# sevagh/xumx-sliCQ

Hardware: AMD Instinct MI355X
Metric: real-time factor (audio-s demixed / wall-s), 44.1 kHz stereo, offline model (higher is better)
Workload: dtype f32; 1 GPU; BASELINE configs[1]: offline model (Bark-262 sliCQT), one 240 s stereo track (10,584,000 samples, 5 chunks) per GPU, Wiener off (mix-phase), seeded synthetic weights; parallelism=one track per rank, 1 rank(s), no data-path collective

## Files before the change

### include/xumx_slicq_hip.h

```cpp
#ifndef XUMX_SLICQ_HIP_H
#define XUMX_SLICQ_HIP_H

#include <stddef.h>
#include <stdint.h>

#ifdef __cplusplus
extern "C" {
#endif

#define XSQ_ABI_VERSION 2

typedef struct xsq_plan xsq_plan;
typedef struct xsq_model xsq_model;

int xsq_abi_version(void);
const char* xsq_last_error(void);
const char* xsq_build_info(void);

int xsq_plan_create(xsq_plan** out, int L, int tr, int nbands, const int32_t* Lg,
                    const int32_t* c, const float* g, const double* gd, const float* tw);
int xsq_plan_destroy(xsq_plan* plan);
int xsq_plan_num_blocks(const xsq_plan* plan);
int xsq_plan_set_fft_backend(xsq_plan* plan, int backend);
int xsq_plan_set_band_radix4(xsq_plan* plan, int on);
int xsq_plan_set_short_inline(xsq_plan* plan, int on);
int xsq_plan_set_packed_fft(xsq_plan* plan, int on);
int xsq_plan_block_table(const xsq_plan* plan, int64_t* table);
int64_t xsq_plan_coefs_per_slice(const xsq_plan* plan);
int xsq_plan_num_slices(const xsq_plan* plan, int64_t n);

size_t xsq_slicqt_forward_workspace(xsq_plan* plan, int BC, int64_t n);
int xsq_slicqt_forward(xsq_plan* plan, const float* x, int BC, int64_t n, float* coef,
                       void* workspace, size_t workspace_bytes, void* stream);
int xsq_slicqt_forward_xin(xsq_plan* plan, const float* x, int BC, int64_t n, float* coef, float* xin,
                           const float* mean, const float* scale, int split,
                           void* workspace, size_t workspace_bytes, void* stream);

int xsq_slicqt_forward_rows(xsq_plan* plan, const float* x, const int64_t* x_row_offsets, int BC, int64_t n,
                            int64_t n_pad, float* coef, float* xin, const float* mean, const float* scale, int split,
                            void* workspace, size_t workspace_bytes, void* stream);
// ... 204 lines not shown
```

### xumx_slicq_amd/_lib.py

```python
from __future__ import annotations

import ctypes as C
import os

import torch

_HERE = os.path.dirname(os.path.abspath(__file__))
LIB_PATH = os.environ.get("XSQ_LIB") or os.path.join(_HERE, "libxumx_slicq_hip.so")


class XsqError(RuntimeError):
    pass


def _load():
    if not os.path.exists(LIB_PATH):
        raise XsqError(
            f"{LIB_PATH} is missing: the HIP extension is the product path and has no CPU "
            "fallback. Build it with `python -c 'import __graft_entry__ as g; g.build()'` "
            "or `make -C xumx_slicq_amd/csrc`.")
    return C.CDLL(LIB_PATH, mode=C.RTLD_GLOBAL)


lib = _load()

_vp = C.c_void_p
_i32p = C.POINTER(C.c_int32)
_i64p = C.POINTER(C.c_int64)

_SIGS = {
    "xsq_abi_version": (C.c_int, []),
    "xsq_last_error": (C.c_char_p, []),
    "xsq_build_info": (C.c_char_p, []),
    "xsq_plan_create": (C.c_int, [C.POINTER(_vp), C.c_int, C.c_int, C.c_int, _vp, _vp, _vp, _vp, _vp]),
    "xsq_plan_destroy": (C.c_int, [_vp]),
    "xsq_plan_num_blocks": (C.c_int, [_vp]),
    "xsq_plan_set_fft_backend": (C.c_int, [_vp, C.c_int]),
    "xsq_plan_set_band_radix4": (C.c_int, [_vp, C.c_int]),
    "xsq_plan_set_short_inline": (C.c_int, [_vp, C.c_int]),
    "xsq_plan_set_packed_fft": (C.c_int, [_vp, C.c_int]),
    "xsq_plan_block_table": (C.c_int, [_vp, _vp]),
    "xsq_plan_coefs_per_slice": (C.c_int64, [_vp]),
    "xsq_plan_num_slices": (C.c_int, [_vp, C.c_int64]),
    "xsq_slicqt_forward_workspace": (C.c_size_t, [_vp, C.c_int, C.c_int64]),
    "xsq_slicqt_forward": (C.c_int, [_vp, _vp, C.c_int, C.c_int64, _vp, _vp, C.c_size_t, _vp]),
    "xsq_slicqt_forward_xin": (C.c_int, [_vp, _vp, C.c_int, C.c_int64, _vp, _vp, _vp, _vp, C.c_int, _vp, C.c_size_t, _vp]),
    "xsq_slicqt_forward_rows": (C.c_int, [_vp, _vp, _vp, C.c_int, C.c_int64, C.c_int64, _vp, _vp, _vp, _vp, C.c_int, _vp, C.c_size_t, _vp]),
    "xsq_slicqt_forward_rows_indirect": (C.c_int, [_vp, _vp, _vp, _vp, C.c_int, C.c_int64, C.c_int64, _vp, _vp, _vp, _vp, C.c_int, _vp, C.c_size_t, _vp]),
    "xsq_slicqt_inverse_workspace": (C.c_size_t, [_vp, C.c_int, C.c_int]),
    "xsq_slicqt_inverse": (C.c_int, [_vp, _vp, C.c_int, C.c_int, C.c_int64, _vp, _vp, C.c_size_t, _vp]),
    "xsq_slicqt_inverse_rows": (C.c_int, [_vp, _vp, C.c_int, C.c_int, C.c_int64, _vp, _vp, _vp, C.c_size_t, _vp]),
    "xsq_slicqt_inverse_masked": (C.c_int, [_vp, _vp, _vp, C.c_int, C.c_int, C.c_int, C.c_int64, _vp, _vp, _vp, C.c_size_t, _vp]),
    "xsq_slicqt_remix_workspace": (C.c_size_t, [_vp, C.c_int, C.c_int, C.c_int, C.c_int]),
    "xsq_slicqt_inverse_remix": (C.c_int, [_vp, _vp, _vp, _vp, _vp, C.c_int, C.c_int, C.c_int, C.c_int64, _vp, _vp, _vp, C.c_size_t, _vp]),
# ... 148 lines not shown
```

### xumx_slicq_amd/csrc/cdae.hip

```cpp
#include <algorithm>
#include <cmath>
#include <cstdlib>
#include <cstring>
#include <vector>

#include "../../include/xumx_slicq_hip.h"
#include "gemm_tile.h"
#include "gemm_tile_bf3.h"
#include "gemm_tile_bf6.h"
#include "plan.h"
#include "prof.h"

#include "cdae_api.h"

namespace xsq {

__global__ __launch_bounds__(256) void k_magnitude_whiten(const float4* __restrict__ X, float4* __restrict__ xin,
                                                           const int64_t* __restrict__ cum,
                                                           const CdaeBlockDev* __restrict__ blocks,
                                                           const float* __restrict__ mean,
                                                           const float* __restrict__ scale, int nblocks,
                                                           int BC, int S, int64_t nquads, int split) {
    __shared__ int64_t cum_s[128];
    for (int i = threadIdx.x; i < nblocks && i < 128; i += 256) cum_s[i] = cum[i];
// ... 860 lines not shown
extern "C" int xsq_debug_w4_stamps(unsigned long long* out, int reset) {
    XSQ_HIP(hipDeviceSynchronize());
    XSQ_HIP(hipMemcpyFromSymbol(out, HIP_SYMBOL(xsq::g_w4_stamps), 8 * sizeof(unsigned long long)));
    if (reset) { unsigned long long z[8] = {0}; XSQ_HIP(hipMemcpyToSymbol(HIP_SYMBOL(xsq::g_w4_stamps), z, sizeof(z))); }
    return XSQ_OK;
}
#endif

int xsq_model_set_wiener_options(xsq_model* Mo, int softmask, int residual) {
    XSQ_REQUIRE(Mo, "xsq_model_set_wiener_options: null model");
    Mo->wiener_flags = (softmask ? XSQ_WIENER_SOFTMASK : 0) | (residual ? XSQ_WIENER_RESIDUAL : 0);
    return XSQ_OK;
}

int xsq_model_set_winograd(xsq_model* Mo, int on) {
    XSQ_REQUIRE(Mo && on >= 0 && on <= 15, "xsq_model_set_winograd: null model or mask %d (1 = layers 2 / 3 Winograd F(2, 4), 2 / 4 = layer 1 / 4 F(2, 2), 8 = F(4, 4) for long rows)", on);
    XSQ_REQUIRE(!(on & 8) || Mo->wino4, "xsq_model_set_winograd: bit 8 (F(4, 4)) needs a model created with XSQ_WINO4=1 in the environment");
    Mo->winograd = on;
    return XSQ_OK;
}

int xsq_model_destroy(xsq_model* Mo) {
    if (!Mo) return XSQ_OK;
    for (auto& kv : Mo->tiles) (void)hipFree(kv.second.d_tiles);
    (void)hipFree(Mo->d_pool); (void)hipFree(Mo->d_upool); (void)hipFree(Mo->d_pool_split); (void)hipFree(Mo->d_mean); (void)hipFree(Mo->d_scale);
    (void)hipFree(Mo->d_blocks); (void)hipFree(Mo->d_cum); (void)hipFree(Mo->d_blockF);
    delete Mo;
    return XSQ_OK;
}

size_t xsq_cdae_workspace(const xsq_model* Mo, int Bn, int S) {
// ... 15 lines not shown
                       (const float4*)X, (float4*)xin, Mo->d_cum, Mo->d_blocks, mean, scale, Mo->nblocks, Bn * 2, S,
                       total / 4, split);
    return XSQ_OK;
}

template <class T>
static void launch_tiles(void (*kernel)(CdaeArgs, const T*, int), int threads, const CdaeArgs& a, const TileTable& tt, hipStream_t stream) {
    if (tt.ntiles) hipLaunchKernelGGL(kernel, dim3(tt.ntiles), dim3(threads), 0, stream, a, (const T*)tt.d_tiles, tt.ntiles);
}

template <bool TRANSPOSED>
static auto slab_kernel(bool bf3, bool bf6) {
    return bf3 ? cdae_slab_kernel<TRANSPOSED, 1> : bf6 ? cdae_slab_kernel<TRANSPOSED, 2> : cdae_slab_kernel<TRANSPOSED, 3, true>;
}

int cdae_launch_layer(xsq_model* Mo, int layer, const CdaeArgs& a, hipStream_t stream, const char* prof_name) {
    if (layer == 1 || layer == 4)
        for (const CdaeBlockDev& d : Mo->blocks)
            XSQ_REQUIRE(std::max((int64_t)4 * 2 * a.Bn * d.F * a.S * d.T, layer == 4 ? (int64_t)4 * CS * a.Bn * a.T1 * d.F1 : 0) < ((int64_t)1 << 30),
                        "xsq_cdae_forward: B=%d S=%d: a block's layer-%d input exceeds 2^30 bytes; split the batch", a.Bn, a.S, layer);
    if (layer == 4 && !a.gx8)
        for (const CdaeBlockDev& d : Mo->blocks)
            XSQ_REQUIRE((int64_t)2 * a.Bn * d.F * a.S * d.T < ((int64_t)1 << 31),
                        "xsq_cdae_forward: B=%d S=%d overflows the 32-bit offsets of a block; split the batch", a.Bn, a.S);
    if (layer == 4 && a.gx8) layer = 6;

    const bool bf3 = a.split != 0;
    const bool bf1 = Mo->precision == 3;
    const bool bf6 = Mo->precision == 2 || bf1;
    const bool inference = !a.raw && !a.xin8 && !a.gx8;
    const bool fp32 = inference && !bf3 && !bf6;
// ... 133 lines not shown
```

### xumx_slicq_amd/csrc/cdae_api.h

```cpp
#pragma once
#include <map>
#include <mutex>
#include <tuple>
#include <vector>

#include "common.h"
#include "plan.h"

namespace xsq {

static const int H1 = 50, H2 = 51, CS = 52;
static const int NT = 4;

struct CdaeBlockDev {
    int F, T, hop, kf, F1, F2;
    int cumF1, cumF2;
    int ld1, ld4;
    int64_t cum;
    int64_t cumF;
    int64_t w1[NT], w2[NT], w3[NT], w4[NT];
    int64_t s1[NT], s2[NT], s3[NT], b4[NT];
    int64_t u2[NT], u3[NT];
    int64_t u1[NT];
    int nch1, pad_;
// ... 34 lines not shown
    const float* pool;
    const float* xin;
    float* act1;
    float* act2;
    float* act3;
    const float* X;
    float* Y;
    float* masks;
    int Bn, S, T1, T2, causal;
    int raw;
    const float* xin8;
    float* gx8;
    int split = 0;
    const float* poolB = nullptr;
    const float* upool = nullptr;
};


int cdae_launch_layer(xsq_model* Mo, int layer, const CdaeArgs& a, hipStream_t stream, const char* prof_name = nullptr);
int cdae_launch_magnitude(const xsq_model* Mo, const float* X, float* xin, const float* mean, const float* scale,
                          int Bn, int S, hipStream_t stream, int split = 0);

int wiener_em_backward(int nblocks, const int32_t* F, const int32_t* T, const float* X, const float* Y0, const float* masks,
                       float* G, int Bn, int S, int win_len, int batch_group, const void* stats, void* bstats, hipStream_t stream,
                       float* gM = nullptr);
int loss_forward_backward(int nblocks, const int32_t* F, const int32_t* T, const float* pred, const float* target,
                          const float* masks, int Bn, int S, double* out, float* gY, float* gM, void* ws, hipStream_t stream);
int sdr_loss(const float* pred, const float* target, int R, int64_t n, float scale, double* out, float* gy, void* ws, hipStream_t stream);

}
// ... 1 lines not shown
```

### xumx_slicq_amd/csrc/cdae_l4f.h

```cpp
#pragma once
#include "cdae_api.h"
#include "gemm_tile.h"

#ifndef XSQ_L4F_WAVES_PER_EU
#define XSQ_L4F_WAVES_PER_EU 3
#endif
#ifndef XSQ_L4F_SCHED
#define XSQ_L4F_SCHED 0
#endif
#ifndef XSQ_L4F_ABL
#define XSQ_L4F_ABL 0
#endif

namespace xsq {

constexpr int L4_PAIRS = 64;
constexpr int L4_BLD = 56;
constexpr int L4_BROWS = 3 * 64;

__host__ __device__ constexpr int l4f_cols(int W) { return (W + 15) / 16 * 16; }
__host__ __device__ constexpr int l4f_tap_floats(int W) { return 3 * CS * l4f_cols(W); }
__host__ __device__ constexpr int l4f_u_off(int W, int n0, int j, int n, int ci) {
    return 3 * CS * n0 + (j * (l4f_cols(W) - n0 < 64 ? l4f_cols(W) - n0 : 64) + (n - n0)) * CS + ci;
}
// ... 202 lines not shown
        load_a(o, addr_of(pr, 0));
        store_b();
        __syncthreads();
        for (int it = 0; it < run; ++it) {
            const bool more = it + 1 < run;
            const Pair nxp = pair_of(more ? it + 1 : it);
            const Addr nx = addr_of(nxp, 0);
            clear_acc();
            contract(o, nx, more);
            epilogue(pr);
            pr = nxp;
        }
        return;
    }
    if constexpr (NCB <= 2) {
        Ops o;
        const Pair pr = pair_of(0);
        clear_acc();
        load_b(0);
        load_a(o, addr_of(pr, 0));
        for (int df = 0; df < kf; ++df) {
            if (df > 0) __syncthreads();
            store_b();
            __syncthreads();
            const bool more = df + 1 < kf;
            if (more) load_b(df + 1);
            contract(o, addr_of(pr, more ? df + 1 : df), more);
        }
        epilogue(pr);
    }
}

template <bool WITH_Y>
__global__ __launch_bounds__(256, XSQ_L4F_WAVES_PER_EU) void cdae_l4f_kernel(CdaeArgs a, const L4fTileDev* __restrict__ tiles, int ntiles) {
#ifndef XSQ_L4F_LDS_ROWS
#define XSQ_L4F_LDS_ROWS L4_BROWS
#endif
    __shared__ __attribute__((aligned(16))) float Bs[XSQ_L4F_LDS_ROWS * L4_BLD];
    const L4fTileDev t = tiles[xcd_remap(blockIdx.x, ntiles)];
    asm volatile("" :: "s"(t.Q0), "s"(t.kf), "s"(t.F), "s"(t.run), "s"(t.in_off), "s"(t.out_off), "s"(t.bias_off), "s"(t.u_off),
// ... 10 lines not shown
```

### xumx_slicq_amd/csrc/cdae_slab.h

```cpp
#pragma once
#include "cdae_api.h"
#include "gemm_tile_bf3.h"
#include "gemm_tile_bf6.h"

#ifndef XSQ_SLAB_PROLOGUE_PRIO
#define XSQ_SLAB_PROLOGUE_PRIO 0
#endif
#ifndef XSQ_SLAB_STAMP
#define XSQ_SLAB_STAMP 0
#endif
#ifndef XSQ_SLAB_PRIO
#define XSQ_SLAB_PRIO 0
#endif
#ifndef XSQ_SLAB_ABL
#define XSQ_SLAB_ABL 0
#endif

namespace xsq {

constexpr int SLAB_ROWS = 256;
constexpr int SLAB_MAXSEG = 4;
constexpr int SLAB_POS = SLAB_ROWS + 3 * SLAB_MAXSEG;
constexpr int SLAB_KRUN = 4 * CS;
constexpr int SLAB_BLD = 36;
// ... 190 lines not shown
    }
    const int b16_frag = (32 + (lane & 15)) * BLD + 4 * q16;
    const int bv_frag = 48 * BLD + 8 * lk;
    f32x4_t acc16[2] = {{0.f, 0.f, 0.f, 0.f}, {0.f, 0.f, 0.f, 0.f}};
    constexpr int NV = TRANSPOSED ? H1 - 48 : H2 - 48;
    float accv[4] = {0.f, 0.f, 0.f, 0.f};

    constexpr int NKS = 7;
#if XSQ_SLAB_PRIO == 1
    if (__builtin_amdgcn_readfirstlane(tid) >= 256) __builtin_amdgcn_s_setprio(1);
#endif
#if XSQ_SLAB_STAMP
    if (a_base == -12345 || a16_base[0] == -12345 || a16_base[1] == -12345 || s_p0 == -12345) __builtin_trap();
    if (TRANSPOSED && tid == 0 && blockIdx.x < SLAB_STAMP_TILES) g_slab_stamps[blockIdx.x * 8 + 7] = __builtin_amdgcn_s_memrealtime();
#endif
    load_slab(0);
    load_b(0, 0, 0);
    XSQ_SS2(1);
#if XSQ_SLAB_STAMP
    if (sa[0].x == 1.2345e-30f) __builtin_trap();
    XSQ_SS2(2);
#endif
    store_slab();
    store_b(0, 0);
#if XSQ_SLAB_STAMP
    stamp_loads = false;
#endif
    load_b(1, 0, 1);
    load_b(0, 0, 2);
    if (kf > 1 && !LATE) load_slab(1);
#if XSQ_SLAB_PROLOGUE_PRIO
    __builtin_amdgcn_s_setprio(0);
#endif
    __syncthreads();
    XSQ_SS(1);
#if XSQ_SLAB_STAMP
    unsigned long long fetch_t = 0;
#endif
    for (int df = 0; df < kf; ++df) {
        const bool more = df + 1 < kf;
#pragma unroll
        for (int ks = 0; ks < 8; ++ks) {
            if (ks < NKS) {
                if constexpr (LATE && EARLY2) { if (ks == NKS - 1 && more) load_slab(df + 1, 0, XSQ_SLAB_EARLY2 == 1 ? 2 : XSQ_SLAB_EARLY2); }
                const unsigned* Bb = Bs + (ks & 1) * SLAB_BN * BLD;
#pragma unroll
                for (int c = 0; c < 2; ++c) {
                    const int k = 32 * ks + 16 * c;
                    if (k < SLAB_KRUN) {
                        if constexpr (MODE == 3) {
#if XSQ_SLAB_PRIO == 2
                            __builtin_amdgcn_s_setprio(1);
#endif
                            const float* Bf = reinterpret_cast<const float*>(Bb);
                            const float4 alo = *reinterpret_cast<const float4*>(&slabF[a_base + k]);
// ... 74 lines not shown
            } else if (more) {
                if constexpr (LATE) {
#if XSQ_SLAB_STAMP
                    const unsigned long long f0 = __builtin_amdgcn_s_memrealtime();
#endif
                    if constexpr (EARLY2) { load_slab(df + 1, XSQ_SLAB_EARLY2 == 1 ? 2 : XSQ_SLAB_EARLY2, NLD); store_slab(0, NLD); }
                    else {
                        load_slab(df + 1, 0, 4); store_slab(0, 4);
                        load_slab(df + 1, 4, NLD); store_slab(4, NLD);
                    }
#if XSQ_SLAB_STAMP
                    fetch_t += __builtin_amdgcn_s_memrealtime() - f0;
#endif
                } else {
                    store_slab();
                    if (df + 2 < kf) load_slab(df + 2);
                }
            }
            if (ks + 1 < NKS) store_b((ks + 1) & 1, (ks + 1) & 1);
            else if (ks + 1 == 8 && more) store_b(0, 0);
            if (ks + 3 < NKS) load_b((ks + 3) & 1, df, ks + 3);
            else if (ks + 3 >= 8 && more) load_b((ks + 3) & 1, df + 1, ks + 3 - 8);
            __syncthreads();
        }
    }
#undef XSQ_MF
    XSQ_SS(2);
#if XSQ_SLAB_STAMP
    if (TRANSPOSED && tid == 0 && blockIdx.x < SLAB_STAMP_TILES) {
        g_slab_stamps[blockIdx.x * 8 + 4] = kf; g_slab_stamps[blockIdx.x * 8 + 5] = fetch_t;
        g_slab_stamps[blockIdx.x * 8 + 6] = (unsigned)__builtin_amdgcn_s_getreg((4) | (0 << 6) | (31 << 11));
// ... 25 lines not shown
```

### xumx_slicq_amd/csrc/cdae_wino.h

```cpp
#pragma once
#include "cdae_api.h"
#include "gemm_tile.h"

#ifndef XSQ_WINO_WAVES_PER_EU
#define XSQ_WINO_WAVES_PER_EU 2
#endif
#ifndef XSQ_WINO_RAW_AHEAD
#define XSQ_WINO_RAW_AHEAD 0
#endif
#ifndef XSQ_WINO_SWAP
#define XSQ_WINO_SWAP 1
#endif
#ifndef XSQ_WINO_SCHED
#define XSQ_WINO_SCHED 0
#endif
#ifndef XSQ_WINO_SCHED2
#define XSQ_WINO_SCHED2 -1
#endif
#ifndef XSQ_WINO_ABL
#define XSQ_WINO_ABL 0
#endif

namespace xsq {

// ... 155 lines not shown
        f.w[2] = *reinterpret_cast<const float4*>(&Bt[bf + 32 * WN_BLD]);
#pragma unroll
        for (int cc = 0; cc < NV; ++cc) f.u[cc] = Bt[bv + cc * WN_BLD];
        if (tail) {
            const int tb = q * WN_BLD + 16 + kq;
            f.wt[0] = Bt[tb]; f.wt[1] = Bt[tb + 16 * WN_BLD]; f.wt[2] = Bt[tb + 32 * WN_BLD];
#pragma unroll
            for (int cc = 0; cc < NV; ++cc) f.ut[cc] = Bt[(48 + cc) * WN_BLD + 16 + kq];
        }
    };

    const int f0 = t.Q0 / P, q0 = t.Q0 - f0 * P;
    const int npairs = min(WN_PAIRS, Fo * P - t.Q0);
    const int n0 = min(npairs, P - q0);
    int cnt = 0;
    load_chunk(0, 0);
    setup_staging(f0, q0, npairs, n0);
    load_slab(0);
    store_slab();
    store_chunk(0, 0);
    __syncthreads();
    WN_STAMP(0);

    {
        const int myseg = pl >= n0 ? 1 : 0;
        const int eb = (pl + 2 * myseg) * WN_SLD + 4 * kq;
        const int ob = PLANE_O + (pl + myseg) * WN_SLD + 4 * kq;
        float4 dn[5];
        auto read_raw = [&](int s) {
            dn[0] = *reinterpret_cast<const float4*>(&slab[eb + 16 * s]);
            dn[1] = *reinterpret_cast<const float4*>(&slab[ob + 16 * s]);
            dn[2] = *reinterpret_cast<const float4*>(&slab[eb + WN_SLD + 16 * s]);
            dn[3] = *reinterpret_cast<const float4*>(&slab[ob + WN_SLD + 16 * s]);
            dn[4] = *reinterpret_cast<const float4*>(&slab[eb + 2 * WN_SLD + 16 * s]);
        };
        clear_acc();
        for (int df = 0; df < kf; ++df) {
            const bool more = df + 1 < kf;
            if (XSQ_WINO_RAW_AHEAD) read_raw(0);
#pragma unroll
            for (int s = 0; s < 3; ++s) {
                const int cur = cnt & 1;
                if (s < 2) load_chunk(df, s + 1);
                else if (more) { load_chunk(df + 1, 0); load_slab(df + 1); }
                const float* Bc = Bs + cur * 5 * WN_BTILE;
                if (!XSQ_WINO_RAW_AHEAD) read_raw(s);
                Frag fr[2];
                read_frag(fr[0], Bc, s == 2);
                float v[5][4], vt[5];
                {
                    const float d[5][4] = {{dn[0].x, dn[0].y, dn[0].z, dn[0].w}, {dn[1].x, dn[1].y, dn[1].z, dn[1].w}, {dn[2].x, dn[2].y, dn[2].z, dn[2].w},
                                           {dn[3].x, dn[3].y, dn[3].z, dn[3].w}, {dn[4].x, dn[4].y, dn[4].z, dn[4].w}};
#pragma unroll
// ... 171 lines not shown
```

### xumx_slicq_amd/csrc/plan.h

```cpp
#pragma once
#include <algorithm>
#include <map>
#include <mutex>
#include <tuple>
#include <vector>

#include <rocfft/rocfft.h>

#include "common.h"

namespace xsq {

struct FftPlan {
    rocfft_plan plan = nullptr;
    rocfft_execution_info info = nullptr;
    size_t work_bytes = 0;
};

struct TileTable {
    TileDev* d_tiles = nullptr;
    int ntiles = 0;
};

enum class TileKind { BandGemm, Dft4Full, CdaeGemm, CdaeSlab, CdaeWino, CdaeL1f, CdaeL4f };
struct TileKey {
    TileKind kind;
    int rows, S;
    int sub, flags;
    bool operator<(const TileKey& o) const {
        return std::tie(kind, rows, S, sub, flags) < std::tie(o.kind, o.rows, o.S, o.sub, o.flags);
    }
};

template <class D, class T>
static int upload(D*& dst, const T* src, size_t count) {
    dst = nullptr;
    if (!count) return XSQ_OK;
    XSQ_HIP(hipMalloc((void**)&dst, count * sizeof(T)));
    const hipError_t e = hipMemcpy(dst, src, count * sizeof(T), hipMemcpyHostToDevice);
// ... 42 lines not shown
    int band_radix4 = 1;
    void* d_bands4 = nullptr;
    float* d_pool4f = nullptr;
    float* d_pool4i = nullptr;
    int nbands4 = 0;
    std::vector<unsigned char> bands4_host;
    int64_t d4_max_block = 0;
    std::vector<int> bands4_m, bands4_small;
    int fft_backend = 0;
    float2* d_T = nullptr;
    unsigned short* d_tgt16 = nullptr;
    int* d_tgt = nullptr;
    int phase_begin[5] = {0, 0, 0, 0, 0};
    int packed_fft = 0;
    int short_inline = 0;
    void *d_s_item1 = nullptr, *d_s_tw1 = nullptr;
    int *d_s_item2 = nullptr, *d_s_tgt = nullptr;
    float* d_s_wd = nullptr;
    int short_n1 = 0, short_n2 = 0, short_nent = 0, short_sc0 = 0;
    int short_begin[5] = {0, 0, 0, 0, 0};
    int phase_long[4] = {0, 0, 0, 0};
    float* d_tw = nullptr;
    float* d_Wf = nullptr;
    float* d_Wi = nullptr;
    xsq::BandDev* d_bands = nullptr;
    int* d_cov_ptr = nullptr;
    int* d_cov_band = nullptr;
    std::vector<int32_t> h_Lg, h_c;
    std::vector<double> h_gd;
    size_t wf_floats = 0, pool4_floats = 0;
// ... 9 lines not shown
```

### xumx_slicq_amd/csrc/slicqt.hip

```cpp
#include <algorithm>
#include <cmath>
#include <cstdarg>
#include <cstdio>
#include <cstdlib>
#include <cstring>

#include "../../include/xumx_slicq_hip.h"
#include "gemm_tile.h"
#include "plan.h"
#include "prof.h"
#include "slice_fft.h"
#include "band_dft4.h"
#include "band_dft4s.h"

namespace xsq {

static thread_local char g_err[1024] = "";
void set_error(const char* fmt, ...) {
    va_list ap;
    va_start(ap, fmt);
    vsnprintf(g_err, sizeof(g_err), fmt, ap);
    va_end(ap);
}

// ... 259 lines not shown
    float* d = a.dst + base * ((int64_t)a.R * a.nch) + (int64_t)ch * per + e;
#pragma unroll
    for (int r = 0; r < 4; ++r) {
        if (r >= a.R) break;
        float4 acc = make_float4(0.f, 0.f, 0.f, 0.f);
#pragma unroll
        for (int t = 0; t < 4; ++t) {
            if (!a.use[t]) continue;
            const float g = a.g[r][t];
            acc.x = acc.x + g * m[t].x; acc.y = acc.y + g * m[t].y; acc.z = acc.z + g * m[t].z; acc.w = acc.w + g * m[t].w;
        }
        *reinterpret_cast<float4*>(d + (int64_t)r * a.nch * per) = acc;
    }
}

static int get_band_tiles(xsq_plan* P, int rows, TileTable* out) {
    const bool r4 = P->band_radix4 && P->nbands4 > 0;
    return cached_tiles<TileDev>(P->mu, P->tiles, TileKey{TileKind::BandGemm, rows, 0, 0, r4 ? 1 : 0}, out, [&](std::vector<TileDev>& t) {
        if (r4) {
            for (int i = (int)P->bands4_small.size() - 1; i >= 0; --i)
                push_group_tiles(t, P->bands4_small[i], rows, 2 * P->bands[P->bands4_small[i]].Lg);
        } else {
            for (int j = P->nbands - 1; j >= 0; --j) push_group_tiles(t, j, rows, 2 * P->bands[j].Lg);
        }
    });
}

#ifndef XSQ_D4_MIN_LG_DEFAULT
#define XSQ_D4_MIN_LG_DEFAULT 24
#endif

struct Switches {
    bool d4_sym = true;
    int d4_min_lg = XSQ_D4_MIN_LG_DEFAULT;
    Switches() {
        if (const char* e = getenv("XSQ_D4_SYM")) d4_sym = atoi(e) != 0;
        if (const char* e = getenv("XSQ_D4_MIN_LG")) d4_min_lg = atoi(e) >= 16 ? atoi(e) : d4_min_lg;
    }
};
static const Switches& switches() { static const Switches sw; return sw; }
// ... 500 lines not shown
    XSQ_HIP(hipMemcpyFromSymbol(host, HIP_SYMBOL(g_fft_stamps), (size_t)(rows < FFT_STAMP_ROWS ? rows : FFT_STAMP_ROWS) * 64));
    return XSQ_OK;
}
#endif

int xsq_plan_set_packed_fft(xsq_plan* P, int on) {
    XSQ_REQUIRE(P, "xsq_plan_set_packed_fft: null plan");
#if !XSQ_PACKED_FFT_KERNELS
    XSQ_REQUIRE(!on, "xsq_plan_set_packed_fft: this library is built without the packed-fp32 slice FFT kernels "
                "(diagnostic build: make PACKED_FFT=1)");
#endif
    P->packed_fft = on ? 1 : 0;
    return XSQ_OK;
}

int xsq_plan_set_short_inline(xsq_plan* P, int on) {
    XSQ_REQUIRE(P, "xsq_plan_set_short_inline: null plan");
    P->short_inline = on ? 1 : 0;
    return XSQ_OK;
}

int xsq_plan_set_fft_backend(xsq_plan* P, int backend) {
    XSQ_REQUIRE(P && (backend == 0 || backend == 1), "xsq_plan_set_fft_backend: backend must be 0 (auto) or 1 (rocFFT)");
    P->fft_backend = backend;
    return XSQ_OK;
}

int xsq_plan_block_table(const xsq_plan* P, int64_t* table) {
    XSQ_REQUIRE(P && table, "xsq_plan_block_table: null argument");
    for (int b = 0; b < P->nblocks; ++b) {
// ... 100 lines not shown
        XSQ_PROF(adj ? "adjoint_slice_rfft" : "slice_rfft", stream);
        auto kernel = k_slice_rfft<512>;
#if XSQ_PACKED_FFT_KERNELS
        if (P->packed_fft) kernel = k_slice_rfft<512, true>;
#endif
        if (ring) kernel = k_slice_rfft<512, false, true>;
        hipLaunchKernelGGL(kernel, dim3(rows), dim3(512), 0, stream, x, d_tw, fft_tables(P), (float2*)U, S, n, P->h, x_rows, x_slot, s0, ring,
                           const_cast<float*>(x), fresh.x, fresh.first, fresh.stride);
    } else {
        { XSQ_PROF(adj ? "adjoint_slice_window" : "slice_window", stream);
        hipLaunchKernelGGL(k_slice_window, dim3((P->L + 255) / 256, rows), dim3(256), 0, stream, x, d_tw, seg,
                           S, n, P->L, P->h, x_rows, x_slot, s0, ring, const_cast<float*>(x), fresh.x, fresh.first, fresh.stride); }
        { XSQ_PROF(adj ? "adjoint_rfft_L" : "rfft_L", stream); rc = run_fft(f, seg, U, fwork, stream); }
        if (rc) return rc;
    }
    TileTable tt;
    rc = get_band_tiles(P, rows, &tt);
    if (rc) return rc;
    BandFwdOp op{U, coef, P->d_bands, d_Wf, BC, S, P->nbins, P->L, xin, mean, scale, split};
    if (P->band_radix4 && P->nbands4) {
        Band4Args a4{(const Band4Dev*)P->d_bands4, d_pool4f, U, coef, BC, S, P->nbins, P->L, 0, nullptr, 0, xin, mean, scale, split};
        XSQ_PROF(adj ? "adjoint_band_dft4" : "band_analysis_dft4", stream);
        if ((rc = launch_dft4<true>(P, a4, rows, 0, stream))) return rc;
    }
    if (tt.ntiles) { XSQ_PROF(adj ? "adjoint_band_gemm" : "band_analysis_gemm", stream);
    hipLaunchKernelGGL((grouped_gemm_kernel<BandFwdOp>), dim3(tt.ntiles), dim3(256), 0, stream, op,
                       tt.d_tiles, tt.ntiles); }
    XSQ_HIP(hipGetLastError());
    return XSQ_OK;
}

int xsq_slicqt_adjoint_window(int L, int nbands, const int32_t* Lg, const int32_t* c, const double* gd, double* out) {
    XSQ_REQUIRE(Lg && c && gd && out, "xsq_slicqt_adjoint_window: null argument");
    XSQ_REQUIRE(L > 0 && L % 4 == 0 && nbands >= 1, "xsq_slicqt_adjoint_window: L=%d nbands=%d", L, nbands);
    int64_t off = 0;
    for (int j = 0; j < nbands; ++j) {
        const int n = Lg[j];
        XSQ_REQUIRE(n > 0 && n % 2 == 0, "xsq_slicqt_adjoint_window: band %d has Lg=%d", j, n);
        for (int q = 0; q < n; ++q) {
            const int k = c[j] + (q < n / 2 ? q : q - n);
            const double w = (k < 0 || k > L / 2) ? 0.0 : ((k == 0 || k == L / 2) ? 1.0 : 2.0);
            out[off + q] = w * (double)n * (double)n * gd[off + q] / (double)L;
// ... 120 lines not shown
    hipStream_t stream = (hipStream_t)stream_;
    const int rows = BC * S;
    FftPlan f;
    int rc = lds_fft(P) ? XSQ_OK : get_fft(P, 1, rows, &f);
    if (rc) return rc;
    char* w = (char*)ws;
    float* Z = (float*)w;    w += al256((size_t)rows * P->sumFT * 8);
    float2* fr = (float2*)w; if (!lds_fft(P)) w += al256((size_t)rows * P->nbins * 8);
    float* seg = (float*)w;  if (!lds_fft(P)) w += al256((size_t)rows * P->L * 4);
    void* fwork = w;
    if ((size_t)(w - (char*)ws) + f.work_bytes > ws_bytes) {
        set_error("xsq_slicqt_inverse: workspace too small (%zu needed, %zu given)",
                  (size_t)(w - (char*)ws) + f.work_bytes, ws_bytes);
        return XSQ_ERR_WORKSPACE;
    }
    TileTable tt;
    rc = get_band_tiles(P, rows, &tt);
    if (rc) return rc;
    BandInvOp op{coef, Z, P->d_bands, P->d_Wi, BC, S, lds_fft(P) ? (int)P->sumFT : 0, mask, BCx};
    if (P->band_radix4 && P->nbands4) {
        Band4Args a4{(const Band4Dev*)P->d_bands4, P->d_pool4i, coef, Z, BC, S, P->nbins, P->L,
                     lds_fft(P) ? (int)P->sumFT : 0, mask, BCx, nullptr, nullptr, nullptr, 0};
        XSQ_PROF("band_synthesis_dft4", stream);
        if ((rc = launch_dft4<false>(P, a4, rows, mask ? BCx * S : 0, stream))) return rc;
    }
    const bool inl = lds_fft(P) && P->band_radix4 && P->short_inline && P->short_n1 > 0 && !carry;
    if (tt.ntiles && !inl) { XSQ_PROF("band_synthesis_gemm", stream);
    hipLaunchKernelGGL((grouped_gemm_kernel<BandInvOp>), dim3(tt.ntiles), dim3(256), 0, stream, op,
                       tt.d_tiles, tt.ntiles); }
    if (lds_fft(P)) {
        XSQ_PROF("slice_irfft_ola", stream);
        GatherSched G;
        G.tgt = P->d_tgt; G.tgt16 = P->d_tgt16; G.row_len = (int)P->sumFT;
        for (int i = 0; i < 5; ++i) G.begin[i] = P->phase_begin[i];
        for (int i = 0; i < 4; ++i) G.lo[i] = inl ? P->phase_long[i] : P->phase_begin[i];
        ShortSched SS;
        memset(&SS, 0, sizeof(SS));
        if (inl) {
            SS.item1 = (const ShortItem1*)P->d_s_item1; SS.tw1 = (const float2*)P->d_s_tw1; SS.item2 = P->d_s_item2;
            SS.stgt = P->d_s_tgt; SS.swd = P->d_s_wd;
            SS.n1 = P->short_n1; SS.n2 = P->short_n2; SS.nent = P->short_nent; SS.sc0 = P->short_sc0;
            for (int i = 0; i < 5; ++i) SS.begin[i] = P->short_begin[i];
        }
        const ShortIn SI{coef, mask, BC, mask ? BCx : BC};
// ... 126 lines not shown
```

### xumx_slicq_amd/transforms.py

```python
from __future__ import annotations

import ctypes as C
from typing import List

import numpy as np
import torch
import torch.nn as nn
from torch import Tensor

from . import _lib
from .arena import BlockTable
from .plan import SliCQPlan, build_plan


def make_filterbanks(nsgt_base, sample_rate=44100.0):
    if sample_rate != 44100.0:
        raise ValueError("i was lazy and harcoded a lot of 44100.0, forgive me")
    return NSGT_SL(nsgt_base), INSGT_SL(nsgt_base)


class SliCQEngine:

    def __init__(self, plan: SliCQPlan):
        self.plan = plan
# ... 20 lines not shown
        for h in self._handles.values():
            _lib.check(_lib.lib.xsq_plan_set_band_radix4(h, int(self._band_radix4)), "xsq_plan_set_band_radix4")

    def set_packed_fft(self, on: bool):
        on = bool(on)
        if on == getattr(self, "_packed_fft", False):
            return
        for h in self._handles.values():
            _lib.check(_lib.lib.xsq_plan_set_packed_fft(h, int(on)), "xsq_plan_set_packed_fft")
        self._packed_fft = on

    def set_short_inline(self, on: bool):
        self._short_inline = bool(on)
        for h in self._handles.values():
            _lib.check(_lib.lib.xsq_plan_set_short_inline(h, int(self._short_inline)), "xsq_plan_set_short_inline")

    def handle(self, device: torch.device):
        if device.type != "cuda":
            raise _lib.XsqError(
                f"the sliCQT runs on a ROCm device only (got a tensor on '{device}'); there is no CPU fallback")
        idx = device.index if device.index is not None else torch.cuda.current_device()
        h = self._handles.get(idx)
        if h is None:
            p = self.plan
            out = C.c_void_p()
            with torch.cuda.device(idx):
                _lib.check(_lib.lib.xsq_plan_create(
                    C.byref(out), p.L, p.tr, p.nbands,
                    p.Lg.ctypes.data, p.c.ctypes.data, p.g.ctypes.data, p.gd.ctypes.data, p.tw.ctypes.data),
                    "xsq_plan_create")
            h = out
            _lib.check(_lib.lib.xsq_plan_set_fft_backend(h, self._fft_backend), "xsq_plan_set_fft_backend")
            _lib.check(_lib.lib.xsq_plan_set_band_radix4(h, int(getattr(self, "_band_radix4", True))),
                       "xsq_plan_set_band_radix4")
            _lib.check(_lib.lib.xsq_plan_set_short_inline(h, int(getattr(self, "_short_inline", False))),
                       "xsq_plan_set_short_inline")
            _lib.check(_lib.lib.xsq_plan_set_packed_fft(h, int(getattr(self, "_packed_fft", False))), "xsq_plan_set_packed_fft")
            self._handles[idx] = h
        return h

    def demixer(self, device: torch.device):
        idx = device.index if device.index is not None else torch.cuda.current_device()
        d = self.__dict__.setdefault("_demixers", {}).get(idx)
        if d is None:
            h = self.handle(device)
            out = C.c_void_p()
            with torch.cuda.device(idx):
                _lib.check(_lib.lib.xsq_demixer_create(C.byref(out), h), "xsq_demixer_create")
            d = self._demixers[idx] = out
        return d

    def workspace(self, device: torch.device, nbytes: int) -> Tensor:
# ... 168 lines not shown
```

Baseline: 55530 x real-time.

## Add register-resident MFMA kernel for short bands and skip dead CDAE border taps

Result: no change. 55890 x real-time (median of 6 runs) (+0.7%).

```diff
diff --git a/include/xumx_slicq_hip.h b/include/xumx_slicq_hip.h
--- a/include/xumx_slicq_hip.h
+++ b/include/xumx_slicq_hip.h
@@ -24,6 +24,7 @@
 int xsq_plan_set_fft_backend(xsq_plan* plan, int backend);
 int xsq_plan_set_band_radix4(xsq_plan* plan, int on);
 int xsq_plan_set_short_inline(xsq_plan* plan, int on);
+int xsq_plan_set_short_mfma(xsq_plan* plan, int on);
 int xsq_plan_set_packed_fft(xsq_plan* plan, int on);
 int xsq_plan_block_table(const xsq_plan* plan, int64_t* table);
 int64_t xsq_plan_coefs_per_slice(const xsq_plan* plan);
diff --git a/xumx_slicq_amd/_lib.py b/xumx_slicq_amd/_lib.py
--- a/xumx_slicq_amd/_lib.py
+++ b/xumx_slicq_amd/_lib.py
@@ -38,6 +38,7 @@
     "xsq_plan_set_fft_backend": (C.c_int, [_vp, C.c_int]),
     "xsq_plan_set_band_radix4": (C.c_int, [_vp, C.c_int]),
     "xsq_plan_set_short_inline": (C.c_int, [_vp, C.c_int]),
+    "xsq_plan_set_short_mfma": (C.c_int, [_vp, C.c_int]),
     "xsq_plan_set_packed_fft": (C.c_int, [_vp, C.c_int]),
     "xsq_plan_block_table": (C.c_int, [_vp, _vp]),
     "xsq_plan_coefs_per_slice": (C.c_int64, [_vp]),
diff --git a/xumx_slicq_amd/csrc/band_short.h b/xumx_slicq_amd/csrc/band_short.h
--- /dev/null
+++ b/xumx_slicq_amd/csrc/band_short.h
@@ -0,0 +1,136 @@
+#pragma once
+#include <type_traits>
+
+#include "common.h"
+#include "gemm_tile.h"
+
+namespace xsq {
+
+constexpr int BS_MAX_LG = 24;
+constexpr int BS_RT = 2;
+constexpr int BS_RUN = 2;
+constexpr int BS_STEP = 64 * BS_RT;
+constexpr int BS_ROWS = BS_STEP * BS_RUN;
+
+template <int NC, class Op>
+__device__ __forceinline__ void band_short_body(const Op& op, const BandDev& b, const int j, const int m0) {
+#pragma clang fp contract(off)
+    constexpr bool FWD = std::is_same<Op, BandFwdOp>::value;
+    const int lane = threadIdx.x & 63, wave = threadIdx.x >> 6;
+    const int q = lane & 15, kq = lane >> 4;
+    const int N = 2 * b.Lg, M = op.BC * op.S, S = op.S;
+    if (m0 + 16 * BS_RT * wave >= M) return;
+
+    float4 w[NC][NC];
+    {
+        const float* W = op.W + b.w_off;
+#pragma unroll
+        for (int nb = 0; nb < NC; ++nb)
+#pragma unroll
+            for (int c = 0; c < NC; ++c)
+                w[nb][c] = 16 * nb + q < N ? *reinterpret_cast<const float4*>(W + (int64_t)(16 * nb + q) * b.ldw + 16 * c + 4 * kq)
+                                           : make_float4(0.f, 0.f, 0.f, 0.f);
+    }
+    float mu = 0.f, sc = 1.f;
+    if constexpr (FWD) { if (op.xin) { mu = op.mean[j]; sc = op.scale[j]; } }
+    const int64_t base = 2 * ((int64_t)op.BC * S * b.cum + (int64_t)b.f * S * b.Lg);
+
+    struct Row { const float* p; const float* mk; int64_t out; bool ok; };
+    auto row_of = [&](int m) {
+        Row r;
+        r.ok = m < M;
+        const int bc = m / S, s = m - bc * S;
+        const int64_t off = base + ((int64_t)bc * b.F * S + s) * N;
+        r.mk = nullptr;
+        if constexpr (FWD) {
+            r.p = op.U + (int64_t)m * 2 * op.nbins;
+            r.out = off;
+        } else {
+            r.out = op.row_len ? 2 * ((int64_t)m * op.row_len + b.ent) : off;
+            if (!op.mask) r.p = op.coef + off;
+            else {
+                r.mk = op.mask + off / 2;
+                r.p = op.coef + 2 * ((int64_t)op.BCx * S * b.cum + (int64_t)b.f * S * b.Lg) + ((int64_t)(bc % op.BCx) * b.F * S + s) * N;
+            }
+        }
+        return r;
+    };
+
+#pragma unroll 1
+    for (int it = 0; it < BS_RUN; ++it) {
+        const int mw = m0 + BS_STEP * it + 16 * BS_RT * wave;
+        if (mw >= M) break;
+        Row r[BS_RT];
+        float4 v[BS_RT][NC];
+        float2 mk[BS_RT][NC];
+#pragma unroll
+        for (int t = 0; t < BS_RT; ++t) {
+            r[t] = row_of(mw + 16 * t + q);
+#pragma unroll
+            for (int c = 0; c < NC; ++c) {
+                const int k = 16 * c + 4 * kq;
+                const bool ok = r[t].ok && k < N;
+                if constexpr (FWD) {
+                    int i0 = b.bin0 + (k >> 1), i1 = i0 + 1;
+                    i0 = i0 < 0 ? -i0 : (i0 > op.L / 2 ? op.L - i0 : i0);
+                    i1 = i1 < 0 ? -i1 : (i1 > op.L / 2 ? op.L - i1 : i1);
+                    const float2 x0 = *reinterpret_cast<const float2*>(ok ? r[t].p + 2 * i0 : zero16());
+                    const float2 x1 = *reinterpret_cast<const float2*>(ok ? r[t].p + 2 * i1 : zero16());
+                    v[t][c] = make_float4(x0.x, x0.y, x1.x, x1.y);
+                } else {
+                    v[t][c] = *reinterpret_cast<const float4*>(ok ? r[t].p + k : zero16());
+                    if (op.mask) mk[t][c] = *reinterpret_cast<const float2*>(ok ? r[t].mk + (k >> 1) : zero16());
+                }
+            }
+        }
+#pragma unroll
+        for (int t = 0; t < BS_RT; ++t) {
+            f32x4 acc[NC];
+#pragma unroll
+            for (int nb = 0; nb < NC; ++nb) acc[nb] = f32x4{0.f, 0.f, 0.f, 0.f};
+#pragma unroll
+            for (int c = 0; c < NC; ++c) {
+                float4 xv = v[t][c];
+                if constexpr (!FWD) {
+                    if (op.mask) { xv.x *= mk[t][c].x; xv.y *= mk[t][c].x; xv.z *= mk[t][c].y; xv.w *= mk[t][c].y; }
+                }
+                const float x[4] = {xv.x, xv.y, xv.z, xv.w};
+#pragma unroll
+                for (int i = 0; i < 4; ++i)
+#pragma unroll
+                    for (int nb = 0; nb < NC; ++nb) {
+                        const float wv[4] = {w[nb][c].x, w[nb][c].y, w[nb][c].z, w[nb][c].w};
+                        acc[nb] = __builtin_amdgcn_mfma_f32_16x16x4f32(wv[i], x[i], acc[nb], 0, 0, 0);
+                    }
+            }
+#pragma unroll
+            for (int nb = 0; nb < NC; ++nb) {
+                const int n = 16 * nb + 4 * kq;
+                if (!r[t].ok || n >= N) continue;
+                const float4 y = make_float4(acc[nb][0], acc[nb][1], acc[nb][2], acc[nb][3]);
+                if constexpr (FWD) {
+                    *reinterpret_cast<float4*>(op.coef + r[t].out + n) = y;
+                    if (op.xin) {
+                        float v0 = whiten_mag(y.x, y.y, mu, sc), v1 = whiten_mag(y.z, y.w, mu, sc);
+                        if (op.split) { v0 = bf3_word(v0); v1 = bf3_word(v1); }
+                        *reinterpret_cast<float2*>(op.xin + ((r[t].out + n) >> 1)) = make_float2(v0, v1);
+                    }
+                } else {
+                    *reinterpret_cast<float4*>(op.Z + r[t].out + n) = y;
+                }
+            }
+        }
+    }
+}
+
+template <class Op>
+__global__ __launch_bounds__(256) void band_short_kernel(const Op op, const TileDev* __restrict__ tiles, int ntiles) {
+    const TileDev t = tiles[blockIdx.x];
+    const BandDev b = op.bands[t.group];
+    const int nc = (2 * b.Lg + 15) >> 4;
+    if (nc == 2) band_short_body<2>(op, b, t.group, t.m0);
+    else if (nc == 3) band_short_body<3>(op, b, t.group, t.m0);
+    else band_short_body<1>(op, b, t.group, t.m0);
+}
+
+}
diff --git a/xumx_slicq_amd/csrc/cdae.hip b/xumx_slicq_amd/csrc/cdae.hip
--- a/xumx_slicq_amd/csrc/cdae.hip
+++ b/xumx_slicq_amd/csrc/cdae.hip
@@ -898,7 +898,8 @@
 }
 
 int xsq_model_set_winograd(xsq_model* Mo, int on) {
-    XSQ_REQUIRE(Mo && on >= 0 && on <= 15, "xsq_model_set_winograd: null model or mask %d (1 = layers 2 / 3 Winograd F(2, 4), 2 / 4 = layer 1 / 4 F(2, 2), 8 = F(4, 4) for long rows)", on);
+    XSQ_REQUIRE(Mo && on >= 0 && on <= 31, "xsq_model_set_winograd: null model or mask %d (1 = layers 2 / 3 Winograd F(2, 4), 2 / 4 = layer 1 / 4 F(2, 2), 8 = F(4, 4) for long rows, "
+                "16 = layers 3 / 4 visit their dead border taps)", on);
     XSQ_REQUIRE(!(on & 8) || Mo->wino4, "xsq_model_set_winograd: bit 8 (F(4, 4)) needs a model created with XSQ_WINO4=1 in the environment");
     Mo->winograd = on;
     return XSQ_OK;
@@ -944,7 +945,9 @@
     return bf3 ? cdae_slab_kernel<TRANSPOSED, 1> : bf6 ? cdae_slab_kernel<TRANSPOSED, 2> : cdae_slab_kernel<TRANSPOSED, 3, true>;
 }
 
-int cdae_launch_layer(xsq_model* Mo, int layer, const CdaeArgs& a, hipStream_t stream, const char* prof_name) {
+int cdae_launch_layer(xsq_model* Mo, int layer, const CdaeArgs& args, hipStream_t stream, const char* prof_name) {
+    CdaeArgs a = args;
+    a.all_taps = (Mo->winograd & 16) ? 1 : 0;
     if (layer == 1 || layer == 4)
         for (const CdaeBlockDev& d : Mo->blocks)
             XSQ_REQUIRE(std::max((int64_t)4 * 2 * a.Bn * d.F * a.S * d.T, layer == 4 ? (int64_t)4 * CS * a.Bn * a.T1 * d.F1 : 0) < ((int64_t)1 << 30),
diff --git a/xumx_slicq_amd/csrc/cdae_api.h b/xumx_slicq_amd/csrc/cdae_api.h
--- a/xumx_slicq_amd/csrc/cdae_api.h
+++ b/xumx_slicq_amd/csrc/cdae_api.h
@@ -72,6 +72,7 @@
     int split = 0;
     const float* poolB = nullptr;
     const float* upool = nullptr;
+    int all_taps = 0;
 };
 
 
diff --git a/xumx_slicq_amd/csrc/cdae_l4f.h b/xumx_slicq_amd/csrc/cdae_l4f.h
--- a/xumx_slicq_amd/csrc/cdae_l4f.h
+++ b/xumx_slicq_amd/csrc/cdae_l4f.h
@@ -240,16 +240,23 @@
         return;
     }
     if constexpr (NCB <= 2) {
+        int df_lo = 0, df_hi = kf - 1;
+        if (!a.all_taps) {
+            const int R0 = t.Q0 / P, R1 = (min(t.Q0 + L4_PAIRS, a.Bn * F * P) - 1) / P;
+            const int b0 = R0 / F, b1 = R1 / F;
+            const int lo = max(0, R0 - b0 * F - F1 + 1), hi = min(kf - 1, R1 - b1 * F);
+            if (b0 == b1 && lo <= hi) { df_lo = lo; df_hi = hi; }
+        }
         Ops o;
         const Pair pr = pair_of(0);
         clear_acc();
-        load_b(0);
-        load_a(o, addr_of(pr, 0));
-        for (int df = 0; df < kf; ++df) {
-            if (df > 0) __syncthreads();
+        load_b(df_lo);
+        load_a(o, addr_of(pr, df_lo));
+        for (int df = df_lo; df <= df_hi; ++df) {
+            if (df > df_lo) __syncthreads();
             store_b();
             __syncthreads();
-            const bool more = df + 1 < kf;
+            const bool more = df < df_hi;
             if (more) load_b(df + 1);
             contract(o, addr_of(pr, more ? df + 1 : df), more);
         }
diff --git a/xumx_slicq_amd/csrc/cdae_slab.h b/xumx_slicq_amd/csrc/cdae_slab.h
--- a/xumx_slicq_amd/csrc/cdae_slab.h
+++ b/xumx_slicq_amd/csrc/cdae_slab.h
@@ -228,8 +228,16 @@
     if (a_base == -12345 || a16_base[0] == -12345 || a16_base[1] == -12345 || s_p0 == -12345) __builtin_trap();
     if (TRANSPOSED && tid == 0 && blockIdx.x < SLAB_STAMP_TILES) g_slab_stamps[blockIdx.x * 8 + 7] = __builtin_amdgcn_s_memrealtime();
 #endif
-    load_slab(0);
-    load_b(0, 0, 0);
+    int df_lo = 0, df_hi = kf - 1;
+    if (TRANSPOSED && !a.all_taps) {
+        int last = 0;
+#pragma unroll
+        for (int i = 1; i < SLAB_MAXSEG; ++i) last += (i * To - t0 < nrows && f0 + i < Fo) ? 1 : 0;
+        const int lo = max(0, f0 - Fi + 1), hi = min(kf - 1, f0 + last);
+        if (lo <= hi) { df_lo = lo; df_hi = hi; }
+    }
+    load_slab(df_lo);
+    load_b(0, df_lo, 0);
     XSQ_SS2(1);
 #if XSQ_SLAB_STAMP
     if (sa[0].x == 1.2345e-30f) __builtin_trap();
@@ -240,9 +248,9 @@
 #if XSQ_SLAB_STAMP
     stamp_loads = false;
 #endif
-    load_b(1, 0, 1);
-    load_b(0, 0, 2);
-    if (kf > 1 && !LATE) load_slab(1);
+    load_b(1, df_lo, 1);
+    load_b(0, df_lo, 2);
+    if (df_lo < df_hi && !LATE) load_slab(df_lo + 1);
 #if XSQ_SLAB_PROLOGUE_PRIO
     __builtin_amdgcn_s_setprio(0);
 #endif
@@ -251,8 +259,8 @@
 #if XSQ_SLAB_STAMP
     unsigned long long fetch_t = 0;
 #endif
-    for (int df = 0; df < kf; ++df) {
-        const bool more = df + 1 < kf;
+    for (int df = df_lo; df <= df_hi; ++df) {
+        const bool more = df < df_hi;
 #pragma unroll
         for (int ks = 0; ks < 8; ++ks) {
             if (ks < NKS) {
@@ -357,7 +365,7 @@
 #endif
                 } else {
                     store_slab();
-                    if (df + 2 < kf) load_slab(df + 2);
+                    if (df + 2 <= df_hi) load_slab(df + 2);
                 }
             }
             if (ks + 1 < NKS) store_b((ks + 1) & 1, (ks + 1) & 1);
diff --git a/xumx_slicq_amd/csrc/cdae_wino.h b/xumx_slicq_amd/csrc/cdae_wino.h
--- a/xumx_slicq_amd/csrc/cdae_wino.h
+++ b/xumx_slicq_amd/csrc/cdae_wino.h
@@ -193,9 +193,14 @@
     const int npairs = min(WN_PAIRS, Fo * P - t.Q0);
     const int n0 = min(npairs, P - q0);
     int cnt = 0;
-    load_chunk(0, 0);
+    int df_lo = 0, df_hi = kf - 1;
+    if (TRANSPOSED && !a.all_taps) {
+        const int lo = max(0, f0 - Fi + 1), hi = min(kf - 1, f0 + (n0 < npairs ? 1 : 0));
+        if (lo <= hi) { df_lo = lo; df_hi = hi; }
+    }
+    load_chunk(df_lo, 0);
     setup_staging(f0, q0, npairs, n0);
-    load_slab(0);
+    load_slab(df_lo);
     store_slab();
     store_chunk(0, 0);
     __syncthreads();
@@ -214,8 +219,8 @@
             dn[4] = *reinterpret_cast<const float4*>(&slab[eb + 2 * WN_SLD + 16 * s]);
         };
         clear_acc();
-        for (int df = 0; df < kf; ++df) {
-            const bool more = df + 1 < kf;
+        for (int df = df_lo; df <= df_hi; ++df) {
+            const bool more = df < df_hi;
             if (XSQ_WINO_RAW_AHEAD) read_raw(0);
 #pragma unroll
             for (int s = 0; s < 3; ++s) {
diff --git a/xumx_slicq_amd/csrc/plan.h b/xumx_slicq_amd/csrc/plan.h
--- a/xumx_slicq_amd/csrc/plan.h
+++ b/xumx_slicq_amd/csrc/plan.h
@@ -22,7 +22,7 @@
     int ntiles = 0;
 };
 
-enum class TileKind { BandGemm, Dft4Full, CdaeGemm, CdaeSlab, CdaeWino, CdaeL1f, CdaeL4f };
+enum class TileKind { BandGemm, BandShort, Dft4Full, CdaeGemm, CdaeSlab, CdaeWino, CdaeL1f, CdaeL4f };
 struct TileKey {
     TileKind kind;
     int rows, S;
@@ -95,6 +95,7 @@
     int phase_begin[5] = {0, 0, 0, 0, 0};
     int packed_fft = 0;
     int short_inline = 0;
+    int short_mfma = 1;
     void *d_s_item1 = nullptr, *d_s_tw1 = nullptr;
     int *d_s_item2 = nullptr, *d_s_tgt = nullptr;
     float* d_s_wd = nullptr;
diff --git a/xumx_slicq_amd/csrc/slicqt.hip b/xumx_slicq_amd/csrc/slicqt.hip
--- a/xumx_slicq_amd/csrc/slicqt.hip
+++ b/xumx_slicq_amd/csrc/slicqt.hip
@@ -297,6 +297,10 @@
     }
 }
 
+}
+#include "band_short.h"
+namespace xsq {
+
 static int get_band_tiles(xsq_plan* P, int rows, TileTable* out) {
     const bool r4 = P->band_radix4 && P->nbands4 > 0;
     return cached_tiles<TileDev>(P->mu, P->tiles, TileKey{TileKind::BandGemm, rows, 0, 0, r4 ? 1 : 0}, out, [&](std::vector<TileDev>& t) {
@@ -307,6 +311,34 @@
             for (int j = P->nbands - 1; j >= 0; --j) push_group_tiles(t, j, rows, 2 * P->bands[j].Lg);
         }
     });
+}
+
+static bool short_stream(const xsq_plan* P) {
+    if (!P->short_mfma || !P->band_radix4 || P->nbands4 <= 0 || P->bands4_small.empty()) return false;
+    for (int j : P->bands4_small) {
+        const BandDev& b = P->bands[j];
+        if (b.Lg % 4 != 0 || b.Lg > BS_MAX_LG || b.ent % 2 != 0 || b.ldw != 16 * ((2 * b.Lg + 15) / 16)) return false;
+    }
+    return true;
+}
+
+static int get_short_tiles(xsq_plan* P, int rows, TileTable* out) {
+    return cached_tiles<TileDev>(P->mu, P->tiles, TileKey{TileKind::BandShort, rows, 0, 0, 0}, out, [&](std::vector<TileDev>& t) {
+        for (int i = (int)P->bands4_small.size() - 1; i >= 0; --i)
+            for (int m0 = 0; m0 < rows; m0 += BS_ROWS) t.push_back(TileDev{P->bands4_small[i], m0, 0, 0});
+    });
+}
+
+template <class Op>
+static int launch_dense_bands(xsq_plan* P, int rows, const Op& op, const char* name, hipStream_t stream) {
+    const bool fast = short_stream(P);
+    TileTable tt;
+    if (int rc = fast ? get_short_tiles(P, rows, &tt) : get_band_tiles(P, rows, &tt)) return rc;
+    if (!tt.ntiles) return XSQ_OK;
+    XSQ_PROF(name, stream);
+    if (fast) hipLaunchKernelGGL((band_short_kernel<Op>), dim3(tt.ntiles), dim3(256), 0, stream, op, tt.d_tiles, tt.ntiles);
+    else hipLaunchKernelGGL((grouped_gemm_kernel<Op>), dim3(tt.ntiles), dim3(256), 0, stream, op, tt.d_tiles, tt.ntiles);
+    return XSQ_OK;
 }
 
 #ifndef XSQ_D4_MIN_LG_DEFAULT
@@ -837,6 +869,12 @@
     return XSQ_OK;
 }
 
+int xsq_plan_set_short_mfma(xsq_plan* P, int on) {
+    XSQ_REQUIRE(P, "xsq_plan_set_short_mfma: null plan");
+    P->short_mfma = on ? 1 : 0;
+    return XSQ_OK;
+}
+
 int xsq_plan_set_short_inline(xsq_plan* P, int on) {
     XSQ_REQUIRE(P, "xsq_plan_set_short_inline: null plan");
     P->short_inline = on ? 1 : 0;
@@ -967,18 +1005,13 @@
         { XSQ_PROF(adj ? "adjoint_rfft_L" : "rfft_L", stream); rc = run_fft(f, seg, U, fwork, stream); }
         if (rc) return rc;
     }
-    TileTable tt;
-    rc = get_band_tiles(P, rows, &tt);
-    if (rc) return rc;
     BandFwdOp op{U, coef, P->d_bands, d_Wf, BC, S, P->nbins, P->L, xin, mean, scale, split};
     if (P->band_radix4 && P->nbands4) {
         Band4Args a4{(const Band4Dev*)P->d_bands4, d_pool4f, U, coef, BC, S, P->nbins, P->L, 0, nullptr, 0, xin, mean, scale, split};
         XSQ_PROF(adj ? "adjoint_band_dft4" : "band_analysis_dft4", stream);
         if ((rc = launch_dft4<true>(P, a4, rows, 0, stream))) return rc;
     }
-    if (tt.ntiles) { XSQ_PROF(adj ? "adjoint_band_gemm" : "band_analysis_gemm", stream);
-    hipLaunchKernelGGL((grouped_gemm_kernel<BandFwdOp>), dim3(tt.ntiles), dim3(256), 0, stream, op,
-                       tt.d_tiles, tt.ntiles); }
+    if ((rc = launch_dense_bands(P, rows, op, adj ? "adjoint_band_gemm" : "band_analysis_gemm", stream))) return rc;
     XSQ_HIP(hipGetLastError());
     return XSQ_OK;
 }
@@ -1129,9 +1162,6 @@
                   (size_t)(w - (char*)ws) + f.work_bytes, ws_bytes);
         return XSQ_ERR_WORKSPACE;
     }
-    TileTable tt;
-    rc = get_band_tiles(P, rows, &tt);
-    if (rc) return rc;
     BandInvOp op{coef, Z, P->d_bands, P->d_Wi, BC, S, lds_fft(P) ? (int)P->sumFT : 0, mask, BCx};
     if (P->band_radix4 && P->nbands4) {
         Band4Args a4{(const Band4Dev*)P->d_bands4, P->d_pool4i, coef, Z, BC, S, P->nbins, P->L,
@@ -1140,9 +1170,7 @@
         if ((rc = launch_dft4<false>(P, a4, rows, mask ? BCx * S : 0, stream))) return rc;
     }
     const bool inl = lds_fft(P) && P->band_radix4 && P->short_inline && P->short_n1 > 0 && !carry;
-    if (tt.ntiles && !inl) { XSQ_PROF("band_synthesis_gemm", stream);
-    hipLaunchKernelGGL((grouped_gemm_kernel<BandInvOp>), dim3(tt.ntiles), dim3(256), 0, stream, op,
-                       tt.d_tiles, tt.ntiles); }
+    if (!inl && (rc = launch_dense_bands(P, rows, op, "band_synthesis_gemm", stream))) return rc;
     if (lds_fft(P)) {
         XSQ_PROF("slice_irfft_ola", stream);
         GatherSched G;
diff --git a/xumx_slicq_amd/transforms.py b/xumx_slicq_amd/transforms.py
--- a/xumx_slicq_amd/transforms.py
+++ b/xumx_slicq_amd/transforms.py
@@ -58,6 +58,11 @@
         self._short_inline = bool(on)
         for h in self._handles.values():
             _lib.check(_lib.lib.xsq_plan_set_short_inline(h, int(self._short_inline)), "xsq_plan_set_short_inline")
+
+    def set_short_mfma(self, on: bool):
+        self._short_mfma = bool(on)
+        for h in self._handles.values():
+            _lib.check(_lib.lib.xsq_plan_set_short_mfma(h, int(self._short_mfma)), "xsq_plan_set_short_mfma")
 
     def handle(self, device: torch.device):
         if device.type != "cuda":
@@ -80,6 +85,7 @@
             _lib.check(_lib.lib.xsq_plan_set_short_inline(h, int(getattr(self, "_short_inline", False))),
                        "xsq_plan_set_short_inline")
             _lib.check(_lib.lib.xsq_plan_set_packed_fft(h, int(getattr(self, "_packed_fft", False))), "xsq_plan_set_packed_fft")
+            _lib.check(_lib.lib.xsq_plan_set_short_mfma(h, int(getattr(self, "_short_mfma", True))), "xsq_plan_set_short_mfma")
             self._handles[idx] = h
         return h
 
```
